# hbell99/DirectVoxGO

Hardware: AMD Instinct MI355X
Metric: train rays/sec (8192-ray batch, 160^3 grid) (higher is better)
Workload: dtype f32

## Files before the change

### directvoxgo_amd/build.py

```python
import os
import subprocess
import sys

HERE = os.path.dirname(os.path.abspath(__file__))
CSRC = os.path.join(HERE, 'csrc')
SO = os.path.join(CSRC, 'libdvgo_hip.so')
SOURCES = ['sampling.hip', 'pointwise.hip', 'composite.hip', 'grid_sample.hip', 'march.hip', 'optim.hip', 'shade.hip', 'shade_x3.hip', 'loss.hip', 'brick.hip', 'maintain.hip', 'metrics.hip', 'mesh.hip', 'shade_pe.hip', 'contract.hip', 'triplane.hip', 'grid_sample_xyz.hip', 'liif.hip', 'plane_rows.hip', 'vm.hip', 'vm_density.hip', 'plane_tv.hip', 'hashgrid.hip']
HEADERS = ['common.h', 'scan.h', 'x3.h', 'xyz_corners.h', 'plane2d.h', 'vm_common.h', os.path.join('..', '..', 'include', 'dvgo_hip.h')]

NO_PACKED_FP32 = ['-fno-slp-vectorize', '-Xclang', '-target-feature', '-Xclang', '-packed-fp32-ops']
FLAGS = ['-O3', '--offload-arch=gfx950', '-std=c++17', '-fPIC', '-shared', '-ffp-contract=off',
         '-munsafe-fp-atomics', '-fno-gpu-rdc', '-Wall', '-Wno-unused-function'] + NO_PACKED_FP32


def needs_build():
    if not os.path.exists(SO):
        return True
    t = os.path.getmtime(SO)
    return any(os.path.getmtime(os.path.join(CSRC, f)) > t for f in SOURCES + HEADERS + [os.path.join('..', 'build.py')])


def build(force=False, verbose=True, extra_flags=()):
    if not force and not needs_build():
        return SO
    hipcc = os.environ.get('HIPCC', '/opt/rocm/bin/hipcc')
    objs = []
    procs = []
    for f in SOURCES:
        o = os.path.join(CSRC, f.replace('.hip', '.o'))
        per_file = os.environ.get('DVGO_FLAGS_' + f.replace('.hip', '').upper(), '').split()
        cmd = [hipcc] + [x for x in FLAGS if x != '-shared'] + list(extra_flags) + per_file + ['-c', os.path.join(CSRC, f), '-o', o]
        if verbose:
            print(' '.join(cmd), flush=True)
        procs.append((cmd, subprocess.Popen(cmd, stderr=subprocess.PIPE, text=True)))
        objs.append(o)
    for cmd, p in procs:
        err = p.communicate()[1]
        err = '\n'.join(ln for ln in err.splitlines() if 'is not a recognized feature for this target' not in ln)
        if err.strip():
            print(err, file=sys.stderr, flush=True)
        if p.returncode != 0:
            raise RuntimeError('hipcc failed: ' + ' '.join(cmd))
    cmd = [hipcc, '--offload-arch=gfx950', '-shared', '-fPIC', '-fno-gpu-rdc', '-o', SO] + objs
    if verbose:
        print(' '.join(cmd), flush=True)
    subprocess.check_call(cmd)
    for o in objs:
        os.remove(o)
    return SO


if __name__ == '__main__':
    build(force='--force' in sys.argv)
    print(SO)
```

### directvoxgo_amd/csrc/march.hip

```cpp
#include <stdlib.h>

#include "common.h"
#include "scan.h"
#include "xyz_corners.h"

__device__ __forceinline__ unsigned long long lanemask_lt(int lane) {
  return (lane == 0) ? 0ull : (~0ull >> (64 - lane));
}


__device__ __forceinline__ float wave_prod_scan(float v, int lane) {
#pragma unroll
  for (int d = 1; d < 64; d <<= 1) {
    const float o = __shfl_up(v, d);
    if (lane >= d) v *= o;
  }
  return v;
}

__device__ __forceinline__ float wave_suffix_excl(float v, int lane, float& total) {
  float inc = v;
#pragma unroll
  for (int d = 1; d < 64; d <<= 1) {
    const float o = __shfl_down(inc, d);
    if (lane + d < 64) inc += o;
  }
  total = dvgo_readlane_f(inc, 0);
  float ex = __shfl_down(inc, 1);
  if (lane == 63) ex = 0.0f;
  return ex;
}

__device__ __forceinline__ int64_t rec_base(const int64_t* __restrict__ cum, const int64_t* __restrict__ n_steps,
                                            int64_t rec_stride, int64_t ray) {
  return cum ? (cum[ray] - n_steps[ray]) : ray * rec_stride;
}

static int g_tuning[DVGO_TUNE_COUNT] = {1, 1, 1, 1, 0, 0, 0, 0};

struct MarchParams {
  float mnx, mny, mnz, mxx, mxy, mxz;
  float stepdist;
  float scx, scy, scz, shx, shy, shz;
  int mX, mY, mZ;
  int X, Y, Z;
  float act_shift, interval, thres;
  int experiment;
};


template <bool FILL>
__device__ __forceinline__ void brick_emit(bool act, int i0, int j0, int k0, int X, int Y, int Z, int lane,
                                           int32_t* __restrict__ cur, int4* __restrict__ recs, const int4 rec) {
  const int BY = (Y + DVGO_BRICK - 1) >> DVGO_BRICK_LOG, BZ = (Z + DVGO_BRICK - 1) >> DVGO_BRICK_LOG;
  int bx0 = 0, bx1 = 0, by0 = 0, by1 = 0, bz0 = 0, bz1 = 0, nx = 0, ny = 0, nz = 0;
  if (act) {
    nx = dvgo_brick_axis(i0, X, bx0, bx1);
    ny = dvgo_brick_axis(j0, Y, by0, by1);
    nz = dvgo_brick_axis(k0, Z, bz0, bz1);
  }
  unsigned pending = (act && nx > 0 && ny > 0 && nz > 0) ? ((1u << (nx * ny * nz)) - 1u) : 0u;
  const unsigned long long lt = lanemask_lt(lane);
  while (__ballot(pending != 0u)) {
    int it = 0, my_id = 0, my_cnt = 0;
    unsigned round = 0u;
    unsigned long long iters = 0ull, ranks = 0ull;
    for (;;) {
      const unsigned long long bal = __ballot(pending != 0u);
      if (!bal || it == 64) break;
      const int leader = __ffsll((long long)bal) - 1;
      const int e = __ffs((int)pending) - 1;
      const int c = (nz == 2) ? (e & 1) : 0, ab = (nz == 2) ? (e >> 1) : e;
      const int b = (ny == 2) ? (ab & 1) : 0, a = (ny == 2) ? (ab >> 1) : ab;
      const int mine = ((a ? bx1 : bx0) << 20) | ((b ? by1 : by0) << 10) | (c ? bz1 : bz0);
      const int Xp = __builtin_amdgcn_readlane(mine, leader);
      const int Xx = Xp >> 20, Xy = (Xp >> 10) & 1023, Xz = Xp & 1023;
      const int ma = (bx0 == Xx) ? 0 : ((nx == 2 && bx1 == Xx) ? 1 : -1);
      const int mb = (by0 == Xy) ? 0 : ((ny == 2 && by1 == Xy) ? 1 : -1);
      const int mc = (bz0 == Xz) ? 0 : ((nz == 2 && bz1 == Xz) ? 1 : -1);
      const bool touch = (pending != 0u) && ma >= 0 && mb >= 0 && mc >= 0;
      const unsigned long long m = __ballot(touch);
      if (lane == it) { my_id = (Xx * BY + Xy) * BZ + Xz; my_cnt = __popcll(m); }
      if (touch) {
        const int em = (((ma << (ny - 1)) + mb) << (nz - 1)) + mc;
        pending &= ~(1u << em);
        round |= 1u << em;
        iters |= (unsigned long long)it << (8 * em);
        ranks |= (unsigned long long)__popcll(m & lt) << (8 * em);
      }
      ++it;
    }
    int base = 0;
    if (lane < it) {
      if (FILL) base = atomicAdd(&cur[my_id], my_cnt);
      else atomicAdd(&cur[my_id], my_cnt);
    }
    if (FILL) {
#pragma unroll
      for (int em = 0; em < 8; ++em) {
        const bool have = (round >> em) & 1u;
        if (!__ballot(have)) continue;
        const int src = (int)((iters >> (8 * em)) & 255ull);
        const int bs = __shfl(base, src);
        if (have) recs[bs + (int)((ranks >> (8 * em)) & 255ull)] = rec;
      }
    }
  }
}

struct MarchTail {
  int32_t* ticket;
  int64_t* off3;
  int32_t *brick_off, *brick_cursor, *extra, *active, *extra_brick;
  int nb, n_extra_max, slice_len;
};

__device__ __forceinline__ int chain_walk(unsigned long long todo, double f, float& Tc, float& T_before) {
  int tc = __builtin_amdgcn_readfirstlane(__float_as_int(Tc));
  int tb = __float_as_int(T_before);
  int sl = -1;
  double d;
  int t;
  asm volatile(
      "s_cmp_eq_u64 %[todo], 0\n\t"
      "s_cbranch_scc1 2f\n"
      "1:\n\t"
      "s_ff1_i32_b64 m0, %[todo]\n\t"
      "s_bitset0_b64 %[todo], m0\n\t"
      "v_cvt_f64_f32 %[d], %[tc]\n\t"
      "v_writelane_b32 %[tb], %[tc], m0\n\t"
      "v_mul_f64 %[d], %[d], %[f]\n\t"
      "v_cvt_f32_f64 %[t], %[d]\n\t"
      "s_nop 0\n\t"
      "v_readlane_b32 %[tc], %[t], m0\n\t"
      "s_cmp_lt_u32 %[tc], 0x3a83126f\n\t"
      "s_cbranch_scc1 3f\n\t"
      "s_cmp_lg_u64 %[todo], 0\n\t"
      "s_cbranch_scc1 1b\n\t"
      "s_branch 2f\n"
      "3:\n\t"
      "s_mov_b32 %[sl], m0\n"
      "2:\n"
      : [todo] "+s"(todo), [tc] "+s"(tc), [tb] "+v"(tb), [sl] "+s"(sl), [d] "=&v"(d), [t] "=&v"(t)
      : [f] "v"(f)
      : "m0", "scc");
  Tc = __int_as_float(tc);
  T_before = __int_as_float(tb);
  return sl;
}

template <bool FAST>
__global__ void __launch_bounds__(DVGO_BLOCK)
march_density_kernel(float* __restrict__ rays_start, float* __restrict__ rays_dir,
                     int64_t* __restrict__ n_steps, const int64_t* __restrict__ cum,
                     int64_t rec_stride, int64_t n_rays, const uint8_t* __restrict__ mask,
                     const float* __restrict__ density, MarchParams P,
                     dvgo_rec2_t* __restrict__ rec2,
                     int32_t* __restrict__ n2, int32_t* __restrict__ n3,
                     float* __restrict__ alphainv_last, int32_t* __restrict__ brick_cnt,
                     const float* __restrict__ rays_o, const float* __restrict__ rays_d, float near, float far, MarchTail tail) {
  const int64_t ray_raw = ((int64_t)blockIdx.x * blockDim.x + threadIdx.x) >> 6;
  const int lane = threadIdx.x & 63;
  const bool live = ray_raw < n_rays;
  const int64_t ray = live ? ray_raw : n_rays - 1;
  if (!live && tail.ticket == nullptr) return;
  int ns;
  float sx, sy, sz, dx, dy, dz;
  if (rays_o != nullptr) {
    const RaySetup R = dvgo_ray_setup(rays_o[3 * ray], rays_o[3 * ray + 1], rays_o[3 * ray + 2], rays_d[3 * ray], rays_d[3 * ray + 1],
                                      rays_d[3 * ray + 2], P.mnx, P.mny, P.mnz, P.mxx, P.mxy, P.mxz, near, far, P.stepdist);
    sx = R.sx; sy = R.sy; sz = R.sz; dx = R.dx; dy = R.dy; dz = R.dz;
    ns = __builtin_amdgcn_readfirstlane((int)R.n);
    if (lane == 0 && live) {
      n_steps[ray] = R.n;
      rays_start[3 * ray] = sx; rays_start[3 * ray + 1] = sy; rays_start[3 * ray + 2] = sz;
      rays_dir[3 * ray] = dx; rays_dir[3 * ray + 1] = dy; rays_dir[3 * ray + 2] = dz;
    }
  } else {
    ns = __builtin_amdgcn_readfirstlane((int)n_steps[ray]);
    sx = rays_start[3 * ray]; sy = rays_start[3 * ray + 1]; sz = rays_start[3 * ray + 2];
    dx = rays_dir[3 * ray]; dy = rays_dir[3 * ray + 1]; dz = rays_dir[3 * ray + 2];
  }
  const int64_t cs0 = (rays_o != nullptr) ? ray * rec_stride : rec_base(cum, n_steps, rec_stride, ray);
  if (!live) ns = 0;
  const int64_t YZ = (int64_t)P.Y * P.Z;
  const bool filt = P.thres > 0.0f;
  const bool pairs = FAST && P.Z >= 2;

  auto probe = [&](int step, float& px, float& py, float& pz, uint8_t& mb) -> bool {
    const float dist = march_dist(P.stepdist, step);
    px = fmaf(dx, dist, sx); py = fmaf(dy, dist, sy); pz = fmaf(dz, dist, sz);
    bool keep = (step < ns) && !((P.mnx > px) | (P.mny > py) | (P.mnz > pz) | (P.mxx < px) | (P.mxy < py) | (P.mxz < pz));
    mb = 1;
    if (mask != nullptr && keep) {
      const int i = (int)roundf(fmaf(px, P.scx, P.shx));
      const int j = (int)roundf(fmaf(py, P.scy, P.shy));
      const int k = (int)roundf(fmaf(pz, P.scz, P.shz));
      keep = (0 <= i) & (i < P.mX) & (0 <= j) & (j < P.mY) & (0 <= k) & (k < P.mZ);
      if (keep && !(P.experiment & 8)) mb = mask[((int64_t)i * P.mY + j) * P.mZ + k];
    }
    return keep;
  };

  float Tc = 1.0f;
  int c2 = 0, c3 = 0;
  float npx = 0.f, npy = 0.f, npz = 0.f;
  uint8_t nmb = 0;
  bool nkeep = false;
  if (FAST) nkeep = probe(lane, npx, npy, npz, nmb);
  for (int base = 0; base < ns; base += 64) {
    const int step = base + lane;
    float px, py, pz;
    bool keep;
    if (FAST) {
      px = npx; py = npy; pz = npz;
      const uint8_t mb = nmb;
      const bool k0 = nkeep;
      if (base + 64 < ns) nkeep = probe(step + 64, npx, npy, npz, nmb);
      keep = k0 && mb != 0;
    } else {
      uint8_t mb;
      keep = probe(step, px, py, pz, mb);
      keep = keep && mb != 0;
    }
    float e = 0.f, a = 0.f;
    TriSetup t;
    t.i0 = t.j0 = t.k0 = 0;
    if (keep) {
      t = dvgo_tri_setup(px, py, pz, P.mnx, P.mny, P.mnz, P.mxx, P.mxy, P.mxz, P.X, P.Y, P.Z);
      float d = 0.f;
      if (P.experiment & 4) {
        d = t.wx0 * 4.0f - 2.0f;
      } else if (pairs) {
        d = dvgo_tri_value_c1(density, t, P.X, P.Y, P.Z);
      } else {
#pragma unroll
        for (int n = 0; n < 8; ++n) {
          if (dvgo_tri_inb(t, n, P.X, P.Y, P.Z)) {
            const int64_t off = (int64_t)(t.i0 + ((n >> 2) & 1)) * YZ + (int64_t)(t.j0 + ((n >> 1) & 1)) * P.Z +
                                (t.k0 + (n & 1));
            d = fmaf(density[off], dvgo_tri_weight(t, n), d);
          }
        }
      }
      if (P.experiment & 2) { e = d * 0.01f; a = e * 0.5f; }
      else {
        e = expf(d + P.act_shift);
        a = 1.0f - dvgo_pow_neg(1.0f + e, -P.interval);
      }
      if (filt) keep = a > P.thres;
    }
    const double f = 1.0 - (double)a + 1e-10;
    float T_before = 1.0f;
    int stop_lane = -1;
    if (P.experiment & 1) {
      T_before = 0.5f;
    } else if (FAST) {
      stop_lane = chain_walk(__ballot(keep), f, Tc, T_before);
    } else {
      unsigned long long todo = __ballot(keep);
      while (todo) {
        const int j = __ffsll((long long)todo) - 1;
        todo &= todo - 1;
        float T_after = 1.0f;
        if (lane == j) { T_before = Tc; T_after = (float)((double)Tc * f); }
        Tc = dvgo_readlane_f(T_after, j);
        if (__float_as_uint(Tc) < 0x3A83126Fu) { stop_lane = j; break; }
      }
    }
    const bool stop = stop_lane >= 0;
    const bool valid2 = keep && (!stop || lane <= stop_lane);
    const float w = T_before * a;
    const bool keep3 = valid2 && (!filt || (w > P.thres));
    const unsigned long long m2 = __ballot(valid2), m3 = __ballot(keep3);
    const unsigned long long lt = lanemask_lt(lane);
    if (valid2) {
      dvgo_rec2_t r;
      r.step = step | (keep3 ? (int32_t)0x80000000 : 0);
      r.exp_d = e; r.alpha = a; r.T = T_before;
      rec2[cs0 + c2 + __popcll(m2 & lt)] = r;
    }
    c2 += __popcll(m2);
    c3 += __popcll(m3);
    if (brick_cnt != nullptr) brick_emit<false>(valid2, t.i0, t.j0, t.k0, P.X, P.Y, P.Z, lane, brick_cnt, nullptr, make_int4(0, 0, 0, 0));
    if (stop) break;
  }
  if (lane == 0 && live) {
    n2[ray] = c2;
    alphainv_last[ray] = Tc;
    if (tail.ticket != nullptr) __hip_atomic_store(&n3[ray], c3, __ATOMIC_RELAXED, __HIP_MEMORY_SCOPE_AGENT);
    else n3[ray] = c3;
  }
  if (tail.ticket == nullptr) return;
  __shared__ int s_is_last;
  asm volatile("s_waitcnt vmcnt(0)" ::: "memory");
  __syncthreads();
  if (threadIdx.x == 0)
    s_is_last = __hip_atomic_fetch_add(tail.ticket, 1, __ATOMIC_RELAXED, __HIP_MEMORY_SCOPE_AGENT) == (int)gridDim.x - 1;
  __syncthreads();
  if (!s_is_last) return;
  block_scan_i32_sc1<DVGO_BLOCK / 64, int64_t>(n3, (int)n_rays, tail.off3);
  if (brick_cnt != nullptr && tail.brick_off != nullptr)
  {
    brick_tables<DVGO_BLOCK / 64, true>(brick_cnt, tail.nb, tail.brick_off, tail.brick_cursor, tail.extra, tail.active,
                                        tail.extra_brick, tail.n_extra_max, tail.slice_len);
    if (threadIdx.x == 0) tail.off3[n_rays + 1] = (int64_t)tail.brick_off[tail.nb];
  }
  if (threadIdx.x == 0) __hip_atomic_store(tail.ticket, 0, __ATOMIC_RELAXED, __HIP_MEMORY_SCOPE_AGENT);
}

__global__ void __launch_bounds__(DVGO_BLOCK)
march_hit_kernel(const float* __restrict__ rays_start, const float* __restrict__ rays_dir,
                 const int64_t* __restrict__ n_steps, int64_t n_rays, const uint8_t* __restrict__ mask, MarchParams P,
                 uint8_t* __restrict__ hit) {
  const int64_t ray = ((int64_t)blockIdx.x * blockDim.x + threadIdx.x) >> 6;
  const int lane = threadIdx.x & 63;
  if (ray >= n_rays) return;
  const int ns = __builtin_amdgcn_readfirstlane((int)n_steps[ray]);
  const float sx = rays_start[3 * ray], sy = rays_start[3 * ray + 1], sz = rays_start[3 * ray + 2];
  const float dx = rays_dir[3 * ray], dy = rays_dir[3 * ray + 1], dz = rays_dir[3 * ray + 2];
  bool any = false;
  for (int base = 0; base < ns && !any; base += 64) {
    const int step = base + lane;
    const float dist = march_dist(P.stepdist, step);
    const float px = fmaf(dx, dist, sx), py = fmaf(dy, dist, sy), pz = fmaf(dz, dist, sz);
    bool keep = (step < ns) && !((P.mnx > px) | (P.mny > py) | (P.mnz > pz) | (P.mxx < px) | (P.mxy < py) | (P.mxz < pz));
    if (keep) {
      const int i = (int)roundf(fmaf(px, P.scx, P.shx));
      const int j = (int)roundf(fmaf(py, P.scy, P.shy));
      const int k = (int)roundf(fmaf(pz, P.scz, P.shz));
      keep = (0 <= i) & (i < P.mX) & (0 <= j) & (j < P.mY) & (0 <= k) & (k < P.mZ);
      if (keep) keep = mask[((int64_t)i * P.mY + j) * P.mZ + k] != 0;
    }
    any = __ballot(keep) != 0ull;
  }
  if (lane == 0) hit[ray] = any ? 1 : 0;
}

template <int CVEC, int CS = 0, int GRP = 1>
__global__ void __launch_bounds__(DVGO_BLOCK)
march_gather_kernel(const dvgo_rec2_t* __restrict__ rec2, const int32_t* __restrict__ n2, const int64_t* __restrict__ n_steps,
                    const int64_t* __restrict__ cum, int64_t rec_stride, const int64_t* __restrict__ off3,
                    int64_t n_rays, const float* __restrict__ rays_start, const float* __restrict__ rays_dir,
                    MarchParams P, const float* __restrict__ k0, int C, int64_t sC, int64_t sX,
                    int64_t sY, int64_t sZ, int64_t* __restrict__ ray_id, int64_t* __restrict__ step_id,
                    float* __restrict__ weights, float* __restrict__ alpha, float* __restrict__ feat) {
  const int64_t r = ((int64_t)blockIdx.x * blockDim.x + threadIdx.x) >> 6;
  const int lane = threadIdx.x & 63;
  if (r >= n_rays) return;
  const int c2 = __builtin_amdgcn_readfirstlane(n2[r]);
  if (c2 == 0) return;
  const int64_t cs0 = rec_base(cum, n_steps, rec_stride, r);
  int64_t out = off3[r];
  const float sx = rays_start[3 * r], sy = rays_start[3 * r + 1], sz = rays_start[3 * r + 2];
  const float dx = rays_dir[3 * r], dy = rays_dir[3 * r + 1], dz = rays_dir[3 * r + 2];
  const unsigned long long lt = lanemask_lt(lane);
  dvgo_rec2_t nrec;
  nrec.step = 0; nrec.exp_d = 0.f; nrec.alpha = 0.f; nrec.T = 0.f;
  if (lane < c2) nrec = rec2[cs0 + lane];
  for (int lo = 0; lo < c2; lo += 64) {
    const int j = lo + lane;
    const dvgo_rec2_t rec = nrec;
    if (j + 64 < c2) nrec = rec2[cs0 + j + 64];
    const bool kept = (j < c2) && (rec.step < 0);
    const unsigned long long m = __ballot(kept);
    const int64_t i = out + __popcll(m & lt);
    out += __popcll(m);
    if (!kept) continue;
    const int step = rec.step & 0x7fffffff;
    ray_id[i] = r;
    step_id[i] = step;
    weights[i] = rec.T * rec.alpha;
    alpha[i] = rec.alpha;
    const float dist = march_dist(P.stepdist, step);
    const float px = fmaf(dx, dist, sx), py = fmaf(dy, dist, sy), pz = fmaf(dz, dist, sz);
    const TriSetup t = dvgo_tri_setup(px, py, pz, P.mnx, P.mny, P.mnz, P.mxx, P.mxy, P.mxz, P.X, P.Y, P.Z);
    float w[8];
    int64_t off[8];
    bool ok[8];
#pragma unroll
    for (int n = 0; n < 8; ++n) {
      w[n] = dvgo_tri_weight(t, n);
      ok[n] = dvgo_tri_inb(t, n, P.X, P.Y, P.Z);
      off[n] = (int64_t)(t.i0 + ((n >> 2) & 1)) * sX + (int64_t)(t.j0 + ((n >> 1) & 1)) * sY +
               (int64_t)(t.k0 + (n & 1)) * sZ;
    }
    if (CVEC > 0) {
      float4 acc[CVEC > 0 ? CVEC : 1];
#pragma unroll
      for (int c = 0; c < CVEC; ++c) acc[c] = make_float4(0.f, 0.f, 0.f, 0.f);
      bool all_in = GRP > 1;
#pragma unroll
      for (int n = 0; n < 8; ++n) all_in = all_in && ok[n];
      if (all_in) {
#pragma unroll
        for (int g = 0; g < 8; g += (GRP > 1 ? GRP : 8)) {
          float4 v[GRP > 1 ? GRP : 1][CVEC > 0 ? CVEC : 1];
#pragma unroll
          for (int n = 0; n < GRP; ++n) {
            const float4* p = reinterpret_cast<const float4*>(k0 + off[g + n]);
#pragma unroll
            for (int c = 0; c < CVEC; ++c) v[n][c] = p[c];
          }
#pragma unroll
          for (int n = 0; n < GRP; ++n) {
#pragma unroll
            for (int c = 0; c < CVEC; ++c) {
              acc[c].x = fmaf(v[n][c].x, w[g + n], acc[c].x);
              acc[c].y = fmaf(v[n][c].y, w[g + n], acc[c].y);
              acc[c].z = fmaf(v[n][c].z, w[g + n], acc[c].z);
              acc[c].w = fmaf(v[n][c].w, w[g + n], acc[c].w);
// ... 371 lines not shown
          }
        }
      }
    }
    if (DEDUP) {
      __builtin_amdgcn_fence(__ATOMIC_SEQ_CST, "workgroup");
#pragma unroll
      for (int it = 0; it < H / 64; ++it) {
        const int s = it * 64 + lane;
        const int k = keys[s];
        if (k != -1) {
          atomicAdd(grad_density + k * gstride, vals[s]);
          keys[s] = -1;
          vals[s] = 0.0f;
        }
      }
      __builtin_amdgcn_fence(__ATOMIC_SEQ_CST, "workgroup");
    }
  }
}

template <int VEC>
__global__ void __launch_bounds__(DVGO_BLOCK)
march_ray_bwd_kernel(const dvgo_rec2_t* __restrict__ rec2, const int32_t* __restrict__ n2,
                     const int64_t* __restrict__ n_steps, const int64_t* __restrict__ cum,
                     int64_t rec_stride, const int64_t* __restrict__ off3, int64_t n_rays,
                     const float* __restrict__ rays_start, const float* __restrict__ rays_dir,
                     MarchParams P, const float* __restrict__ alphainv_last,
                     const float* __restrict__ rays_o, const float* __restrict__ rays_d, float near, float far,
                     const float* __restrict__ density, const float* __restrict__ k0, int C, int64_t sC, int64_t sX,
                     int64_t sY, int64_t sZ, const float* __restrict__ grad_weights,
                     const float* __restrict__ grad_last, const float* __restrict__ grad_feat,
                     float* __restrict__ grad_o, float* __restrict__ grad_d) {
  const int64_t ray = ((int64_t)blockIdx.x * blockDim.x + threadIdx.x) >> 6;
  const int lane = threadIdx.x & 63;
  if (ray >= n_rays) return;
  const int c2 = __builtin_amdgcn_readfirstlane(n2[ray]);
  float Ax = 0.f, Ay = 0.f, Az = 0.f, Bx = 0.f, By = 0.f, Bz = 0.f;
  if (c2 > 0) {
    const int64_t cs0 = rec_base(cum, n_steps, rec_stride, ray);
    const int64_t o3 = off3[ray];
    int c3_rem = (int)(off3[ray + 1] - o3);
    const float sx = rays_start[3 * ray], sy = rays_start[3 * ray + 1], sz = rays_start[3 * ray + 2];
    const float dx = rays_dir[3 * ray], dy = rays_dir[3 * ray + 1], dz = rays_dir[3 * ray + 2];
    const RaySetup R = dvgo_ray_setup(rays_o[3 * ray], rays_o[3 * ray + 1], rays_o[3 * ray + 2], rays_d[3 * ray], rays_d[3 * ray + 1],
                                      rays_d[3 * ray + 2], P.mnx, P.mny, P.mnz, P.mxx, P.mxy, P.mxz, near, far, P.stepdist);
    const int64_t YZ = (int64_t)P.Y * P.Z;
    const float scale_x = (float)(P.X - 1) / (P.mxx - P.mnx);
    const float scale_y = (float)(P.Y - 1) / (P.mxy - P.mny);
    const float scale_z = (float)(P.Z - 1) / (P.mxz - P.mnz);
    const unsigned long long lt = lanemask_lt(lane);
    float acc = (grad_last ? grad_last[ray] : 0.0f) * alphainv_last[ray];
    for (int hi = c2; hi > 0; hi -= 64) {
      const int lo = max(0, hi - 64);
      const int n = hi - lo;
      const bool act = lane < n;
      dvgo_rec2_t rec;
      rec.step = 0; rec.exp_d = 0.f; rec.alpha = 0.f; rec.T = 0.f;
      if (act) rec = rec2[cs0 + lo + lane];
      const bool flag = act && (rec.step < 0);
      const int step = rec.step & 0x7fffffff;
      const unsigned long long m = __ballot(flag);
      const int cnt = __popcll(m);
      const int rank = c3_rem - cnt + __popcll(m & lt);
      c3_rem -= cnt;
      const float gw = flag ? grad_weights[o3 + rank] : 0.0f;
      const float w = rec.T * rec.alpha;
      float total;
      const float suffix = wave_suffix_excl(gw * w, lane, total);
      const float my_acc = acc + suffix;
      acc += total;
      float gx = 0.f, gy = 0.f, gz = 0.f, lam = 0.f;
      if (act) {
        const float gt = gw * rec.T;
        const float one_minus = 1.0f - rec.alpha;
        const float g_alpha = (float)((double)gt - (double)my_acc / ((double)one_minus + 1e-10));
        double v = fmin((double)rec.exp_d, 1e10) * (double)dvgo_pow_neg(1.0f + rec.exp_d, -P.interval - 1.0f);
        v = v * (double)P.interval;
        v = v * (double)g_alpha;
        const float g_d = (float)v;
        const float dist = march_dist(P.stepdist, step);
        const float px = fmaf(dx, dist, sx), py = fmaf(dy, dist, sy), pz = fmaf(dz, dist, sz);
        const TriSetup t = dvgo_tri_setup(px, py, pz, P.mnx, P.mny, P.mnz, P.mxx, P.mxy, P.mxz, P.X, P.Y, P.Z);
        const bool feat = flag && grad_feat != nullptr && C > 0;
        if (g_d != 0.0f || feat) {
          const XyzCorners k = dvgo_xyz_corners(t, P.X, P.Y, P.Z, YZ, (int64_t)P.Z, 1);
          float ax = 0.f, ay = 0.f, az = 0.f;
          {
            float dv[8];
#pragma unroll
            for (int c = 0; c < 8; ++c) dv[c] = density[k.off[c]];
            __builtin_amdgcn_sched_barrier(0);
            DVGO_XYZ_CHANNEL(dv[n], g_d);
          }
          if (feat) {
            int64_t koff[8];
#pragma unroll
            for (int c = 0; c < 8; ++c) {
              const int i = min(max(t.i0 + ((c >> 2) & 1), 0), P.X - 1);
              const int j = min(max(t.j0 + ((c >> 1) & 1), 0), P.Y - 1);
              const int kk = min(max(t.k0 + (c & 1), 0), P.Z - 1);
              koff[c] = (int64_t)i * sX + (int64_t)j * sY + (int64_t)kk * sZ;
            }
            const float* __restrict__ grow = grad_feat + (o3 + rank) * (int64_t)C;
            if (VEC == 4) {
              for (int c = 0; c < C; c += 4) {
                float4 fv[8];
#pragma unroll
                for (int q = 0; q < 8; ++q) fv[q] = *reinterpret_cast<const float4*>(k0 + koff[q] + c);
                const float4 g = *reinterpret_cast<const float4*>(grow + c);
                __builtin_amdgcn_sched_barrier(0);
                DVGO_XYZ_CHANNEL(fv[n].x, g.x);
                DVGO_XYZ_CHANNEL(fv[n].y, g.y);
                DVGO_XYZ_CHANNEL(fv[n].z, g.z);
                DVGO_XYZ_CHANNEL(fv[n].w, g.w);
              }
            } else {
              for (int c = 0; c < C; ++c) {
                float fv[8];
#pragma unroll
                for (int q = 0; q < 8; ++q) fv[q] = k0[c * sC + koff[q]];
                const float g = grow[c];
                DVGO_XYZ_CHANNEL(fv[n], g);
              }
            }
          }
          gx = ax * scale_x; gy = ay * scale_y; gz = az * scale_z;
          lam = R.tmin + dist / R.rnorm;
        }
      }
      Ax += wave_sum(gx); Ay += wave_sum(gy); Az += wave_sum(gz);
      Bx += wave_sum(lam * gx); By += wave_sum(lam * gy); Bz += wave_sum(lam * gz);
    }
  }
  if (lane == 0) {
    grad_o[3 * ray] = Ax; grad_o[3 * ray + 1] = Ay; grad_o[3 * ray + 2] = Az;
    grad_d[3 * ray] = Bx; grad_d[3 * ray + 1] = By; grad_d[3 * ray + 2] = Bz;
  }
}

static MarchParams make_params(const float* mn, const float* mx, float stepdist, const float* sc,
                               const float* sh, int mX, int mY, int mZ, int X, int Y, int Z,
                               float act_shift, float interval, float thres) {
  MarchParams P;
  P.mnx = mn[0]; P.mny = mn[1]; P.mnz = mn[2];
  P.mxx = mx[0]; P.mxy = mx[1]; P.mxz = mx[2];
  P.stepdist = stepdist;
  P.scx = sc ? sc[0] : 0.f; P.scy = sc ? sc[1] : 0.f; P.scz = sc ? sc[2] : 0.f;
  P.shx = sh ? sh[0] : 0.f; P.shy = sh ? sh[1] : 0.f; P.shz = sh ? sh[2] : 0.f;
  P.mX = mX; P.mY = mY; P.mZ = mZ;
  P.X = X; P.Y = Y; P.Z = Z;
  P.act_shift = act_shift; P.interval = interval; P.thres = thres;
  P.experiment = g_tuning[DVGO_TUNE_EXPERIMENT];
  return P;
}

extern "C" {

int dvgo_set_tuning(int key, int value) {
  if (key < 0 || key >= DVGO_TUNE_COUNT) return DVGO_EINVAL;
  g_tuning[key] = value;
  return 0;
}


int dvgo_march_density(float* rays_start, float* rays_dir, int64_t* n_steps,
                       const int64_t* n_steps_cumsum, int64_t rec_stride, int64_t n_rays, const float* xyz_min,
                       const float* xyz_max, float stepdist, const uint8_t* mask, int mX, int mY, int mZ,
                       const float* xyz2ijk_scale, const float* xyz2ijk_shift, const float* density,
                       int X, int Y, int Z, float act_shift, float interval, float fast_color_thres,
                       dvgo_rec2_t* rec2, int32_t* n2, int32_t* n3,
                       float* alphainv_last, int32_t* brick_cnt, const float* rays_o, const float* rays_d, float near,
                       float far, int32_t* tail_ticket, int64_t* off3, int n_bricks, int32_t* brick_off, int32_t* brick_cursor,
                       int32_t* extra_off, int32_t* active, int32_t* extra_brick, int n_extra_max, int slice_len, void* stream) {
  if (n_rays < 0 || X <= 0 || Y <= 0 || Z <= 0) return DVGO_EINVAL;
  if (n_rays == 0) return 0;
  if (!rays_start || !rays_dir || !n_steps || !xyz_min || !xyz_max || !density ||
      !rec2 || !n2 || !n3 || !alphainv_last)
    return DVGO_EINVAL;
  if (!n_steps_cumsum && rec_stride <= 0) return DVGO_EINVAL;
  if (rays_o && (!rays_d || rec_stride <= 0 || stepdist <= 0.0f)) return DVGO_EINVAL;
  if (mask && (!xyz2ijk_scale || !xyz2ijk_shift || mX <= 0 || mY <= 0 || mZ <= 0)) return DVGO_EINVAL;
  if (!dvgo_fits(n_rays * 64)) return DVGO_ERANGE;
  const MarchParams P = make_params(xyz_min, xyz_max, stepdist, xyz2ijk_scale, xyz2ijk_shift, mX, mY, mZ,
                                    X, Y, Z, act_shift, interval, fast_color_thres);
  MarchTail tail;
  tail.ticket = tail_ticket; tail.off3 = off3;
  tail.brick_off = brick_off; tail.brick_cursor = brick_cursor; tail.extra = extra_off; tail.active = active;
  tail.extra_brick = extra_brick; tail.nb = n_bricks; tail.n_extra_max = n_extra_max; tail.slice_len = slice_len;
  if (tail_ticket) {
    if (!off3 || n_rays >= ((int64_t)1 << 31)) return DVGO_EINVAL;
    if (brick_cnt && brick_off && (!brick_cursor || n_bricks <= 0)) return DVGO_EINVAL;
    if (brick_cnt && brick_off && extra_off && (!active || !extra_brick || n_extra_max < 0 || slice_len < 256 || n_bricks >= (1 << 18)))
      return DVGO_EINVAL;
  }
  if (g_tuning[DVGO_TUNE_DENSITY_FWD])
    march_density_kernel<true><<<dvgo_blocks(n_rays * 64, DVGO_BLOCK), DVGO_BLOCK, 0, (hipStream_t)stream>>>(
        rays_start, rays_dir, n_steps, n_steps_cumsum, rec_stride, n_rays, mask, density, P, rec2, n2, n3,
        alphainv_last, brick_cnt, rays_o, rays_d, near, far, tail);
  else
    march_density_kernel<false><<<dvgo_blocks(n_rays * 64, DVGO_BLOCK), DVGO_BLOCK, 0, (hipStream_t)stream>>>(
        rays_start, rays_dir, n_steps, n_steps_cumsum, rec_stride, n_rays, mask, density, P, rec2, n2, n3,
        alphainv_last, brick_cnt, rays_o, rays_d, near, far, tail);
  DVGO_LAUNCH_CHECK();
  return 0;
}

int dvgo_march_hit(const float* rays_start, const float* rays_dir, const int64_t* n_steps, int64_t n_rays,
                   const float* xyz_min, const float* xyz_max, float stepdist, const uint8_t* mask, int mX, int mY,
                   int mZ, const float* xyz2ijk_scale, const float* xyz2ijk_shift, uint8_t* hit, void* stream) {
  if (n_rays < 0) return DVGO_EINVAL;
  if (n_rays == 0) return 0;
  if (!rays_start || !rays_dir || !n_steps || !xyz_min || !xyz_max || !mask || !xyz2ijk_scale || !xyz2ijk_shift || !hit ||
      mX <= 0 || mY <= 0 || mZ <= 0)
    return DVGO_EINVAL;
  if (!dvgo_fits(n_rays * 64)) return DVGO_ERANGE;
  const MarchParams P = make_params(xyz_min, xyz_max, stepdist, xyz2ijk_scale, xyz2ijk_shift, mX, mY, mZ, 1, 1, 1, 0.f, 0.f, 0.f);
  march_hit_kernel<<<dvgo_blocks(n_rays * 64, DVGO_BLOCK), DVGO_BLOCK, 0, (hipStream_t)stream>>>(
      rays_start, rays_dir, n_steps, n_rays, mask, P, hit);
  DVGO_LAUNCH_CHECK();
  return 0;
}

int dvgo_march_gather(const dvgo_rec2_t* rec2, const int32_t* n2, const int64_t* n_steps, const int64_t* n_steps_cumsum,
                      int64_t rec_stride, const int64_t* off3, int64_t n_rays, int64_t M3, const float* rays_start,
                      const float* rays_dir, float stepdist, const float* xyz_min, const float* xyz_max,
                      const float* k0, int C, int X, int Y, int Z, int64_t sC, int64_t sX, int64_t sY,
                      int64_t sZ, int64_t* ray_id, int64_t* step_id, float* weights, float* alpha,
                      float* feat, void* stream) {
  if (n_rays < 0 || M3 < 0 || C < 0 || X <= 0 || Y <= 0 || Z <= 0) return DVGO_EINVAL;
  if (M3 == 0 || n_rays == 0) return 0;
  if (!rec2 || !n2 || !n_steps || !off3 || !rays_start || !rays_dir || !xyz_min || !xyz_max ||
      !ray_id || !step_id || !weights || !alpha || (C > 0 && (!k0 || !feat)))
    return DVGO_EINVAL;
  if (!n_steps_cumsum && rec_stride <= 0) return DVGO_EINVAL;
  if (!dvgo_fits(n_rays * 64)) return DVGO_ERANGE;
  const MarchParams P = make_params(xyz_min, xyz_max, stepdist, nullptr, nullptr, 0, 0, 0, X, Y, Z, 0.f, 0.f, 0.f);
  hipStream_t s = (hipStream_t)stream;
  const int blocks = dvgo_blocks(n_rays * 64, DVGO_BLOCK);
  const bool vec = (sC == 1) && (C % 4 == 0) && (sX % 4 == 0) && (sY % 4 == 0) && (sZ % 4 == 0) &&
                   ((((uintptr_t)k0) & 15) == 0) && ((((uintptr_t)feat) & 15) == 0);
#define DVGO_GATHER(CV, CSS, G)                                                                                      \
  march_gather_kernel<CV, CSS, G><<<blocks, DVGO_BLOCK, 0, s>>>(rec2, n2, n_steps, n_steps_cumsum, rec_stride, off3, \
      n_rays, rays_start, rays_dir, P, k0, C, sC, sX, sY, sZ, ray_id, step_id, weights, alpha, feat)
  const int grp = g_tuning[DVGO_TUNE_GATHER];
  if (vec && C == 12 && grp == 8) DVGO_GATHER(3, 0, 8);
  else if (vec && C == 12 && grp >= 1) DVGO_GATHER(3, 0, 4);
  else if (vec && C == 12) DVGO_GATHER(3, 0, 1);
  else if (vec && C == 4) DVGO_GATHER(1, 0, 8);
  else if (vec && C == 8) DVGO_GATHER(2, 0, 4);
  else if (vec && C == 16) DVGO_GATHER(4, 0, 4);
  else if (sC == 1 && C == 9) DVGO_GATHER(0, 9, 1);
  else if (sC == 1 && C == 3) DVGO_GATHER(0, 3, 1);
  else DVGO_GATHER(0, 0, 1);
#undef DVGO_GATHER
  DVGO_LAUNCH_CHECK();
  return 0;
}

int dvgo_march_composite(const float* weights, const float* rgb, const int64_t* step_id,
                         const int64_t* off3, int64_t n_rays, const float* alphainv_last, float bg,
                         float* rgb_marched, float* depth, void* stream) {
  if (n_rays < 0) return DVGO_EINVAL;
  if (n_rays == 0) return 0;
  if (!off3 || !alphainv_last || !rgb_marched) return DVGO_EINVAL;
  if (!dvgo_fits(n_rays * 64)) return DVGO_ERANGE;
  march_composite_kernel<<<dvgo_blocks(n_rays * 64, DVGO_BLOCK), DVGO_BLOCK, 0, (hipStream_t)stream>>>(
      weights, rgb, step_id, off3, n_rays, alphainv_last, bg, rgb_marched, depth);
  DVGO_LAUNCH_CHECK();
  return 0;
}

int dvgo_march_composite_bwd(const float* grad_rgb_marched, const float* weights, const float* rgb,
                             const int64_t* ray_id, int64_t M3, const int64_t* m_dev, int64_t n_rays, float bg,
                             float* grad_weights, float* grad_rgb, float* grad_last, int accumulate, void* stream) {
  if (M3 < 0 || n_rays < 0) return DVGO_EINVAL;
  const int64_t n_last = grad_last ? n_rays : 0;
  if (M3 == 0 && n_last == 0) return 0;
  if (!grad_rgb_marched || (M3 > 0 && (!weights || !rgb || !ray_id))) return DVGO_EINVAL;
  const int64_t threads = M3 > n_last ? M3 : n_last;
  if (!dvgo_fits(threads)) return DVGO_ERANGE;
  march_composite_bwd_kernel<<<dvgo_blocks(threads, DVGO_BLOCK), DVGO_BLOCK, 0, (hipStream_t)stream>>>(
      grad_rgb_marched, weights, rgb, ray_id, M3, m_dev, grad_weights, grad_rgb, n_last, bg, grad_last, accumulate);
  DVGO_LAUNCH_CHECK();
  return 0;
}

int dvgo_march_feat_bwd(const float* grad_feat, const float* grad_extra, const int64_t* ray_id, const int64_t* step_id,
                        int64_t M3, const float* rays_start, const float* rays_dir, float stepdist,
                        const float* xyz_min, const float* xyz_max, int C, int X, int Y, int Z,
                        int64_t sC, int64_t sX, int64_t sY, int64_t sZ, float* grad_k0, void* stream) {
  if (M3 < 0 || C < 0 || X <= 0 || Y <= 0 || Z <= 0) return DVGO_EINVAL;
  if (M3 == 0 || C == 0) return 0;
  if (!grad_feat || !ray_id || !step_id || !rays_start || !rays_dir || !xyz_min || !xyz_max || !grad_k0)
    return DVGO_EINVAL;
  if (!dvgo_fits(M3 * C)) return DVGO_ERANGE;
  const MarchParams P = make_params(xyz_min, xyz_max, stepdist, nullptr, nullptr, 0, 0, 0, X, Y, Z, 0.f, 0.f, 0.f);
  hipStream_t s = (hipStream_t)stream;
  const int variant = g_tuning[DVGO_TUNE_FEAT_BWD];
  const bool rows = (sC == 1) && (sZ >= C) && (sY == (int64_t)Z * sZ) && (sX == (int64_t)Y * Z * sZ) &&
                    ((int64_t)X * Y * Z < ((int64_t)1 << 31)) && ((C % 4 != 0) || ((((uintptr_t)grad_feat) & 15) == 0));
  const int RS = (int)sZ;
  const int64_t n_pass = (M3 + 31) / 32;
  const int blocks = (int)((n_pass + 3) / 4 < 4096 ? (n_pass + 3) / 4 : 4096);
#define DVGO_FEAT_BWD(CC, EX)                                                                             \
  march_feat_bwd_dedup_kernel<CC, EX><<<blocks, DVGO_BLOCK, 0, s>>>(grad_feat, grad_extra, ray_id, step_id, M3, rays_start, \
// ... 109 lines not shown
```

### include/dvgo_hip.h

```cpp
#ifndef DVGO_HIP_H
#define DVGO_HIP_H

#include <stdint.h>

#ifdef __cplusplus
extern "C" {
#endif

#define DVGO_EINVAL (-1)
#define DVGO_ERANGE (-2)

#define DVGO_ABI_VERSION 11
int dvgo_abi_version(void);

#define DVGO_TUNE_FEAT_BWD    0
#define DVGO_TUNE_DENSITY_BWD 1
#define DVGO_TUNE_DENSITY_FWD 2
#define DVGO_TUNE_GATHER      3
#define DVGO_TUNE_EXPERIMENT  4
#define DVGO_TUNE_COUNT       8
int dvgo_set_tuning(int key, int value);

int dvgo_infer_t_minmax(const float* rays_o, const float* rays_d,
                        const float* xyz_min, const float* xyz_max,
                        float near, float far, int64_t n_rays,
                        float* t_min, float* t_max, void* stream);

int dvgo_infer_n_samples(const float* t_min, const float* t_max, float stepdist,
                         int64_t n_rays, int64_t* n_samples, void* stream);

int dvgo_infer_ray_start_dir(const float* rays_o, const float* rays_d, const float* t_min,
                             int64_t n_rays, float* rays_start, float* rays_dir, void* stream);

int dvgo_sample_pts_prepare(const float* rays_o, const float* rays_d,
                            const float* xyz_min, const float* xyz_max,
                            float near, float far, float stepdist, int64_t n_rays,
                            float* t_min, float* t_max,
                            int64_t* n_steps,
                            int64_t* n_steps_cumsum,
                            float* rays_start, float* rays_dir,
                            void* stream);

int dvgo_sample_pts_fill(const float* rays_start, const float* rays_dir,
                         const float* xyz_min, const float* xyz_max,
                         const int64_t* n_steps_cumsum, int64_t n_rays,
                         float stepdist, int64_t total_len,
                         float* rays_pts,
                         uint8_t* mask_outbbox,
                         int64_t* ray_id, int64_t* step_id,
                         void* stream);

int dvgo_sample_ndc_pts_on_rays(const float* rays_o, const float* rays_d,
                                const float* xyz_min, const float* xyz_max,
                                int n_samples, int64_t n_rays,
                                float* rays_pts, uint8_t* mask_outbbox, void* stream);

int dvgo_maskcache_lookup(const uint8_t* world, const float* xyz,
                          const float* xyz2ijk_scale, const float* xyz2ijk_shift,
                          int sz_i, int sz_j, int sz_k, int64_t n_pts,
                          uint8_t* out, void* stream);

int dvgo_raw2alpha(const float* density, float shift, float interval, int64_t n_pts,
                   float* exp_d, float* alpha, void* stream);
int dvgo_raw2alpha_backward(const float* exp_d, const float* grad_back, float interval,
                            int64_t n_pts, float* grad, void* stream);

int dvgo_alpha2weight(const float* alpha, const int64_t* ray_id, int64_t n_pts, int64_t n_rays,
                      float* weight, float* T, float* alphainv_last,
                      int64_t* i_start, int64_t* i_end, void* stream);
int dvgo_alpha2weight_backward(const float* alpha, const float* weight, const float* T,
                               const float* alphainv_last, const int64_t* i_start,
                               const int64_t* i_end, int64_t n_rays, int64_t n_pts,
                               const float* grad_weights, const float* grad_last,
                               float* grad , void* stream);

int dvgo_grid_sample_fwd(const float* grid, int C, int X, int Y, int Z,
                         int64_t sC, int64_t sX, int64_t sY, int64_t sZ,
                         const float* xyz, const float* xyz_min, const float* xyz_max,
                         int64_t M, float* out, void* stream);
int dvgo_grid_sample_bwd(const float* grad_out, int C, int X, int Y, int Z,
                         int64_t sC, int64_t sX, int64_t sY, int64_t sZ,
                         const float* xyz, const float* xyz_min, const float* xyz_max,
                         int64_t M, float* grad_grid, void* stream);

int dvgo_segment_sum(const float* src, const int64_t* index, int64_t M, int C,
                     int64_t N, float* out, void* stream);

typedef struct { int32_t step; float exp_d; float alpha; float T; } dvgo_rec2_t;

int dvgo_march_density(float* rays_start, float* rays_dir,
                       int64_t* n_steps, const int64_t* n_steps_cumsum, int64_t rec_stride,
                       int64_t n_rays,
                       const float* xyz_min, const float* xyz_max, float stepdist,
                       const uint8_t* mask, int mX, int mY, int mZ,
                       const float* xyz2ijk_scale, const float* xyz2ijk_shift,
                       const float* density, int X, int Y, int Z,
                       float act_shift, float interval, float fast_color_thres,
                       dvgo_rec2_t* rec2,
                       int32_t* n2, int32_t* n3, float* alphainv_last,
                       int32_t* brick_cnt ,
                       const float* rays_o, const float* rays_d, float near, float far
                                          ,
                       int32_t* tail_ticket ,
                       int64_t* off3, int n_bricks, int32_t* brick_off, int32_t* brick_cursor, int32_t* extra_off,
                       int32_t* active, int32_t* extra_brick, int n_extra_max, int slice_len,
                       void* stream);

int dvgo_march_hit(const float* rays_start, const float* rays_dir, const int64_t* n_steps, int64_t n_rays,
                   const float* xyz_min, const float* xyz_max, float stepdist,
                   const uint8_t* mask, int mX, int mY, int mZ,
                   const float* xyz2ijk_scale, const float* xyz2ijk_shift, uint8_t* hit, void* stream);

int dvgo_exclusive_scan_i32(const int32_t* counts, int64_t n, int64_t* offsets, void* stream);

int dvgo_march_gather(const dvgo_rec2_t* rec2, const int32_t* n2, const int64_t* n_steps, const int64_t* n_steps_cumsum,
                      int64_t rec_stride, const int64_t* off3, int64_t n_rays, int64_t M3,
                      const float* rays_start, const float* rays_dir, float stepdist,
                      const float* xyz_min, const float* xyz_max,
                      const float* k0, int C, int X, int Y, int Z,
                      int64_t sC, int64_t sX, int64_t sY, int64_t sZ,
                      int64_t* ray_id, int64_t* step_id, float* weights, float* alpha,
                      float* feat, void* stream);

int dvgo_march_composite(const float* weights, const float* rgb ,
                         const int64_t* step_id, const int64_t* off3, int64_t n_rays,
                         const float* alphainv_last, float bg,
                         float* rgb_marched , float* depth ,
                         void* stream);

int dvgo_march_composite_bwd(const float* grad_rgb_marched , const float* weights,
                             const float* rgb, const int64_t* ray_id, int64_t M3, const int64_t* m_dev, int64_t n_rays,
                             float bg, float* grad_weights , float* grad_rgb ,
                             float* grad_last, int accumulate, void* stream);

int dvgo_march_feat_bwd(const float* grad_feat, const float* grad_extra, const int64_t* ray_id, const int64_t* step_id,
                        int64_t M3, const float* rays_start, const float* rays_dir, float stepdist,
                        const float* xyz_min, const float* xyz_max,
                        int C, int X, int Y, int Z, int64_t sC, int64_t sX, int64_t sY, int64_t sZ,
                        float* grad_k0, void* stream);

int dvgo_march_density_bwd(const dvgo_rec2_t* rec2, const int32_t* n2, const int64_t* n_steps,
                           const int64_t* n_steps_cumsum, int64_t rec_stride, const int64_t* off3,
                           int64_t n_rays,
                           const float* rays_start, const float* rays_dir, float stepdist,
                           const float* xyz_min, const float* xyz_max,
                           const float* alphainv_last, float interval,
                           const float* grad_weights , const float* grad_last ,
                           int X, int Y, int Z, float* grad_density, int64_t grad_stride, float* grad_kept,
                           int32_t* brick_cursor, void* brick_recs,
                           void* stream);

int dvgo_march_ray_bwd(const dvgo_rec2_t* rec2, const int32_t* n2, const int64_t* n_steps,
                       const int64_t* n_steps_cumsum, int64_t rec_stride, const int64_t* off3, int64_t n_rays,
                       const float* rays_start, const float* rays_dir, float stepdist,
                       const float* xyz_min, const float* xyz_max, const float* alphainv_last, float interval,
                       const float* rays_o, const float* rays_d, float near, float far,
                       const float* density, int X, int Y, int Z,
                       const float* k0, int C, int64_t sC, int64_t sX, int64_t sY, int64_t sZ,
                       const float* grad_weights , const float* grad_last ,
                       const float* grad_feat , float* grad_o, float* grad_d, void* stream);

int dvgo_n_bricks(int X, int Y, int Z);
int dvgo_brick_slice(void);
int dvgo_brick_scan(int32_t* brick_cnt, int n_bricks, int32_t* brick_off, int32_t* brick_cursor, int32_t* extra_off,
                    int32_t* active, int32_t* extra_brick , int n_extra_max, int slice_len, void* stream);
int dvgo_march_scans(const int32_t* n3, int64_t n_rays, int64_t* off3, int32_t* brick_cnt, int n_bricks,
                     int32_t* brick_off, int32_t* brick_cursor, int32_t* extra_off, int32_t* active, int32_t* extra_brick,
                     int n_extra_max, int slice_len, void* stream);
int dvgo_brick_accumulate(const int32_t* brick_off, const int32_t* extra_off, const int32_t* active,
                          const int32_t* extra_brick, int32_t* arrive, float* scratch, int64_t n_extra_max, int slice_len,
                          const void* recs, const float* rays_start, const float* rays_dir,
                          float stepdist, const float* xyz_min, const float* xyz_max, const float* grad_feat,
// ... 208 lines not shown
```

Baseline: 3.029 million.

## Add systolic DPP wave-shift transmittance carry with adaptive selection over serial chain walk

Adds an alternative way to compute the exclusive transmittance product across a wavefront. Each lane repeatedly takes its left neighbour's value through a DPP wave_shr:1 move and multiplies it by its own factor in double precision, in unrolled blocks of 16 steps. A heuristic picks this systolic path over the serial per-active-lane chain walk when the span of kept lanes is small compared with their count. The new tuning key is on by default in adaptive mode, and the hand-written asm with s_nop hazard padding adds exposure to DPP hazard rules.

```diff
diff --git a/directvoxgo_amd/build.py b/directvoxgo_amd/build.py
--- a/directvoxgo_amd/build.py
+++ b/directvoxgo_amd/build.py
@@ -6,7 +6,7 @@
 CSRC = os.path.join(HERE, 'csrc')
 SO = os.path.join(CSRC, 'libdvgo_hip.so')
 SOURCES = ['sampling.hip', 'pointwise.hip', 'composite.hip', 'grid_sample.hip', 'march.hip', 'optim.hip', 'shade.hip', 'shade_x3.hip', 'loss.hip', 'brick.hip', 'maintain.hip', 'metrics.hip', 'mesh.hip', 'shade_pe.hip', 'contract.hip', 'triplane.hip', 'grid_sample_xyz.hip', 'liif.hip', 'plane_rows.hip', 'vm.hip', 'vm_density.hip', 'plane_tv.hip', 'hashgrid.hip']
-HEADERS = ['common.h', 'scan.h', 'x3.h', 'xyz_corners.h', 'plane2d.h', 'vm_common.h', os.path.join('..', '..', 'include', 'dvgo_hip.h')]
+HEADERS = ['common.h', 'lane_shift.h', 'scan.h', 'x3.h', 'xyz_corners.h', 'plane2d.h', 'vm_common.h', os.path.join('..', '..', 'include', 'dvgo_hip.h')]
 
 NO_PACKED_FP32 = ['-fno-slp-vectorize', '-Xclang', '-target-feature', '-Xclang', '-packed-fp32-ops']
 FLAGS = ['-O3', '--offload-arch=gfx950', '-std=c++17', '-fPIC', '-shared', '-ffp-contract=off',
diff --git a/directvoxgo_amd/csrc/lane_shift.h b/directvoxgo_amd/csrc/lane_shift.h
--- /dev/null
+++ b/directvoxgo_amd/csrc/lane_shift.h
@@ -0,0 +1,9 @@
+#pragma once
+
+#define DVGO_WAVE_SHR1(dst, src) "v_mov_b32_dpp " dst ", " src " wave_shr:1 row_mask:0xf bank_mask:0xf\n\t"
+
+__device__ __forceinline__ int dvgo_wave_shr1(int v, int first) {
+  int r = first;
+  asm volatile("s_nop 4\n\t" DVGO_WAVE_SHR1("%0", "%1") : "+v"(r) : "v"(v));
+  return r;
+}
diff --git a/directvoxgo_amd/csrc/march.hip b/directvoxgo_amd/csrc/march.hip
--- a/directvoxgo_amd/csrc/march.hip
+++ b/directvoxgo_amd/csrc/march.hip
@@ -1,6 +1,7 @@
 #include <stdlib.h>
 
 #include "common.h"
+#include "lane_shift.h"
 #include "scan.h"
 #include "xyz_corners.h"
 
@@ -36,7 +37,7 @@
   return cum ? (cum[ray] - n_steps[ray]) : ray * rec_stride;
 }
 
-static int g_tuning[DVGO_TUNE_COUNT] = {1, 1, 1, 1, 0, 0, 0, 0};
+static int g_tuning[DVGO_TUNE_COUNT] = {1, 1, 1, 1, 0, 2, 0, 0};
 
 struct MarchParams {
   float mnx, mny, mnz, mxx, mxy, mxz;
@@ -46,6 +47,7 @@
   int X, Y, Z;
   float act_shift, interval, thres;
   int experiment;
+  int carry;
 };
 
 
@@ -149,6 +151,45 @@
   return sl;
 }
 
+#define DVGO_REP4(X) X X X X
+#define DVGO_REP16(X) DVGO_REP4(DVGO_REP4(X))
+constexpr int DVGO_CARRY_BLOCK = 16;
+__device__ __forceinline__ int chain_systolic(unsigned long long todo, double f, int lane, float& Tc, float& T_before) {
+  const int lo = __ffsll((long long)todo) - 1, hi = 63 - __clzll((long long)todo);
+  const double g = ((todo >> lane) & 1ull) ? f : 1.0;
+  int n = hi - lo + 1;
+  int tin = __float_as_int(Tc), t = tin;
+  double d;
+  asm volatile(
+      "s_nop 4\n"
+      "1:\n\t"
+      DVGO_REP16(
+      DVGO_WAVE_SHR1("%[tin]", "%[t]")
+      "v_cvt_f64_f32 %[d], %[tin]\n\t"
+      "v_mul_f64 %[d], %[d], %[g]\n\t"
+      "v_cvt_f32_f64 %[t], %[d]\n\t"
+      "s_nop 1\n\t")
+      "s_sub_i32 %[n], %[n], 16\n\t"
+      "s_cmp_gt_i32 %[n], 0\n\t"
+      "s_cbranch_scc1 1b\n"
+      : [tin] "+v"(tin), [t] "+v"(t), [n] "+s"(n), [d] "=&v"(d)
+      : [g] "v"(g)
+      : "scc");
+  static_assert(DVGO_CARRY_BLOCK == 16, "the asm body above is one block");
+  const unsigned long long below = __ballot((unsigned)t < 0x3A83126Fu) & todo;
+  const int sl = below ? __ffsll((long long)below) - 1 : -1;
+  Tc = __int_as_float(__builtin_amdgcn_readlane(t, sl >= 0 ? sl : hi));
+  T_before = __int_as_float(tin);
+  return sl;
+}
+
+__device__ __forceinline__ bool carry_systolic(int mode, unsigned long long todo) {
+  if (mode != 2) return mode == 1;
+  const unsigned span = (unsigned)((63 - __clzll((long long)todo)) - (__ffsll((long long)todo) - 1) + 1);
+  const unsigned iters = (span + DVGO_CARRY_BLOCK - 1u) & ~(DVGO_CARRY_BLOCK - 1u);
+  return 5u * iters + 12u < 12u * (unsigned)__popcll(todo);
+}
+
 template <bool FAST>
 __global__ void __launch_bounds__(DVGO_BLOCK)
 march_density_kernel(float* __restrict__ rays_start, float* __restrict__ rays_dir,
@@ -256,7 +297,9 @@
     if (P.experiment & 1) {
       T_before = 0.5f;
     } else if (FAST) {
-      stop_lane = chain_walk(__ballot(keep), f, Tc, T_before);
+      const unsigned long long todo = __ballot(keep);
+      if (todo != 0ull && carry_systolic(P.carry, todo)) stop_lane = chain_systolic(todo, f, lane, Tc, T_before);
+      else stop_lane = chain_walk(todo, f, Tc, T_before);
     } else {
       unsigned long long todo = __ballot(keep);
       while (todo) {
@@ -934,6 +977,7 @@
   P.X = X; P.Y = Y; P.Z = Z;
   P.act_shift = act_shift; P.interval = interval; P.thres = thres;
   P.experiment = g_tuning[DVGO_TUNE_EXPERIMENT];
+  P.carry = g_tuning[DVGO_TUNE_CARRY];
   return P;
 }
 
diff --git a/include/dvgo_hip.h b/include/dvgo_hip.h
--- a/include/dvgo_hip.h
+++ b/include/dvgo_hip.h
@@ -18,6 +18,7 @@
 #define DVGO_TUNE_DENSITY_FWD 2
 #define DVGO_TUNE_GATHER      3
 #define DVGO_TUNE_EXPERIMENT  4
+#define DVGO_TUNE_CARRY       5
 #define DVGO_TUNE_COUNT       8
 int dvgo_set_tuning(int key, int value);
 
```

After: 3.044 million, median of 6. No clear change (+0.5%).
